# owensgroup/rtx_nerf

Hardware: AMD Instinct MI355X
Metric: Mrays/sec rendered (NeRF inference render, traverse->sample->MLP->composite) (higher is better)
Workload: dtype f16; 1 GPU; 800x800 inference render, 128^3 grid (procedural Lego stand-in occupancy, 5.3% cells), 8x128 ReLU MLP + Composite-Frequency encoding, 32 samples/segment, 4 hemisphere poses, seeded random fp16 weights; parallelism=single GPU, trace_mode=dda+mip, segments_per_frame_local_max=3152993

## Files before the change

### rtx_nerf_amd/csrc/mlp.hip

```cpp
#include "common.h"

#include <cmath>
#include <cstdlib>
#include <cstring>
#include <mutex>
#include <type_traits>
#include <vector>

#include "mlp_internal.h"

namespace {

#ifndef RTXN_SHARE_DIR
#define RTXN_SHARE_DIR 1
#endif
using rtxn::stage;

struct FwdArgs {
  const uint8_t* packed;
  int n_hidden;
  int out_act;
  const float* input;
  long n;
  const float* start;
  const float* end;
  const float* seg_view;
  const int* total_segments;
  long max_segments;
  _Float16* out_half;
  float4* radiance;
  float* t_vals;
};

struct Enc16Dims { int PD, PF, DD, DF, E, k0; };
__host__ __device__ inline int enc16_feature(const Enc16Dims& d, int u, int g) {
  const int FBD = (d.DF + 3) / 4, FBP = (d.PF + 3) / 4, ND = d.DD * FBD, NP = d.PD * FBP;
  const int width = 2 * (d.PD * d.PF + d.DD * d.DF);
  const int D = u >> 1, ph = u & 1;
  if (D < ND) { const int dd = D / FBD, f = FBD * g + D % FBD; return f < d.DF ? 2 * d.PD * d.PF + (dd * d.DF + f) * 2 + ph : -1; }
  if (D < ND + NP) { const int v = D - ND, dim = v / FBP, f = FBP * g + v % FBP; return f < d.PF ? (dim * d.PF + f) * 2 + ph : -1; }
  const int feat = width + 4 * (2 * (D - ND - NP) + ph) + g;
  return feat < d.E ? feat : -1;
}

__global__ void pack16_kernel(const _Float16* __restrict__ params, _Float16* __restrict__ packed, int W, int n_hidden, Enc16Dims d) {
  const int RT = W / 16, KS = W / 32, KS0 = d.k0 / 32, E = d.E;
  const long l0 = (long)KS0 * RT * 512, hid = (long)KS * RT * 512, outl = 4L * KS * 512;
  const long total = l0 + (long)(n_hidden - 1) * hid + outl;
  for (long e = (long)blockIdx.x * blockDim.x + threadIdx.x; e < total; e += (long)gridDim.x * blockDim.x) {
    int layer;
    long q = e;
    if (q < l0) layer = 0;
    else {
      q -= l0;
      layer = 1 + (int)(q / hid);
      if (layer >= n_hidden) { layer = n_hidden; q -= (long)(n_hidden - 1) * hid; } else q -= (long)(layer - 1) * hid;
    }
// ... 56 lines not shown
      const int feat = rtxn::perm_feature(kk, h, j);
      if (row < rows && feat < in_w) v = params[src_base(layer) + (long)row * in_w + feat];
    } else {
      const int ks_count = layer == n_hidden ? 1 : W / 16;
      const int kk = (int)(chunk % ks_count), rt = (int)(chunk / ks_count);
      const int col = 32 * rt + r;
      const int row = rtxn::perm_feature(kk, h, j);
      if (row < rows && col < in_w) v = params[src_base(layer) + (long)row * in_w + col];
    }
    packed[e] = v;
  }
}

template <int PD, int PF, int DD, int DF>
struct EncSpec16 {
  static constexpr int FBP = (PF + 3) / 4, FBD = (DF + 3) / 4;
  static_assert(FBP >= 1 && FBP <= 3 && FBD >= 1 && FBD <= 3, "octave_unit is written for 1-3 octaves per block");
  static constexpr int enc_width = 2 * (PD * PF + DD * DF);
  static constexpr int enc_padded = (enc_width + 15) / 16 * 16;
  static constexpr int ND = DD * FBD, NP = PD * FBP;
  static constexpr int NPADW = (enc_padded - enc_width + 7) / 8;
  static constexpr int n_dwords = ND + NP + NPADW;
  static constexpr int k0 = (n_dwords + 3) / 4 * 32;
  static_assert(ND <= 8, "direction dwords are placed before the pipeline starts: k-steps 0 and 1 only");
};

template <int NK>
__device__ __forceinline__ void octave_unit(float xg, int (&d)[3]) {
  float t, u, sn, cs;
  if constexpr (NK == 3) {
    asm volatile(
        "v_fract_f32 %3, %7\n\t"
        "v_sin_f32 %5, %3\n\t"
        "v_cos_f32 %6, %3\n\t"
        "s_nop 0\n\t"
        "v_cvt_pk_f16_f32 %0, %5, %6\n\t"
        "v_add_f32 %3, %5, %5\n\t"
        "v_mul_f32 %4, %3, %6\n\t"
        "v_fma_f32 %6, -%3, %5, 1.0\n\t"
// ... 40 lines not shown
template <int PD, int PF, int DD, int DF>
__device__ __forceinline__ void share_direction16(const float (&dir_g)[DD], int lane, int (&dirs)[DirShare16<PD, PF, DD, DF>::n_dwords]) {
  constexpr int FBD = EncSpec16<PD, PF, DD, DF>::FBD;
  const int c = lane & 15;
  float xs = dir_g[0];
#pragma unroll
  for (int dd = 1; dd < DD; ++dd) xs = c == dd ? dir_g[dd] : xs;
  int d[3];
  octave_unit<FBD>(xs, d);
#pragma unroll
  for (int dd = 0; dd < DD; ++dd)
#pragma unroll
    for (int k = 0; k < FBD; ++k) dirs[dd * FBD + k] = __builtin_amdgcn_ds_bpermute(4 * ((lane & 48) + dd), d[k]);
}

template <class ES, int PD, int PF, int DD, int DF, int KS0, int NB, int CT, bool SHARE>
__device__ __forceinline__ void encode_layer0_input(const float (&xq)[CT][5], const int (&dirs)[CT / 2][DirShare16<PD, PF, DD, DF>::n_dwords],
                                                    half8 (&bf)[NB][CT]) {
#pragma unroll
  for (int ct = 0; ct < CT; ++ct) {
    rtxn::int4v t[KS0];
#pragma unroll
    for (int kk = 0; kk < KS0; ++kk)
#pragma unroll
      for (int e = 0; e < 4; ++e) {
        const int D = 4 * kk + e;
        t[kk][e] = (D >= ES::ND + ES::NP && D < ES::n_dwords) ? 0x3c003c00 : 0;
      }
    if constexpr (SHARE) {
#pragma unroll
      for (int D = 0; D < ES::ND; ++D) t[D / 4][D % 4] = dirs[ct / 2][D];
    } else {
#pragma unroll
      for (int dd = 0; dd < DD; ++dd) {
        int d[3];
        octave_unit<ES::FBD>(xq[ct][PD + dd], d);
#pragma unroll
        for (int k = 0; k < ES::FBD; ++k) t[(dd * ES::FBD + k) / 4][(dd * ES::FBD + k) % 4] = d[k];
      }
    }
#pragma unroll
    for (int dim = 0; dim < PD; ++dim) {
      int d[3];
      octave_unit<ES::FBP>(xq[ct][dim], d);
#pragma unroll
      for (int k = 0; k < ES::FBP; ++k) t[(ES::ND + ES::FBP * dim + k) / 4][(ES::ND + ES::FBP * dim + k) % 4] = d[k];
    }
#pragma unroll
    for (int kk = 0; kk < KS0; ++kk) bf[kk][ct] = __builtin_bit_cast(half8, t[kk]);
    if constexpr (SHARE) asm volatile("" : "+v"(bf[0][ct]));
  }
}

#ifdef RTXN_STAMPS
constexpr int kStampTiles = 4, kStampSlots = 24;
__device__ unsigned g_stamps[8 * kStampTiles * kStampSlots];
#define RTXN_STAMP(k)                                                                                     \
  do {                                                                                                    \
    if (blockIdx.x == 0 && tile_it >= 2 && tile_it < 2 + kStampTiles) {                                   \
      const unsigned t_ = (unsigned)__builtin_amdgcn_s_memtime();                                         \
      if (lane == 0) stamp_lds[(wave_u * kStampTiles + (tile_it - 2)) * kStampSlots + (k)] = t_;          \
    }                                                                                                     \
  } while (0)
#else
#define RTXN_STAMP(k)
#endif
// ... 27 lines not shown
  } else {
    n_tiles = (int)((a.n + TILE - 1) / TILE);
  }
  n_tiles = __builtin_amdgcn_readfirstlane(n_tiles);
  const int tile_step = (int)gridDim.x;
  if ((int)blockIdx.x >= n_tiles) return;

  const int n_layers = a.n_hidden + 1;
  auto layer_off = [&](int l) -> unsigned { return l == 0 ? 0u : (unsigned)L0_BYTES + (unsigned)(l - 1) * HID_BYTES; };
  const int grp = wave_u >> 2;
  const int n_hid = n_layers - 2;
  stage<L0_BYTES, THREADS>(a.packed, smem, tid);
  stage<OUT_BYTES, THREADS>(a.packed + layer_off(n_layers - 1), smem + L0_BYTES, tid);
  int qs = 0;

  const float pos_scale = 0.5f * (float)(1u << (ES::FBP * g)), dir_scale = 0.5f * (float)(1u << (ES::FBD * g));
  float xq[CT][5];
  auto sample_of = [&](int tile, int ct, bool& valid) -> long {
    if (IN_MODE == 1) {
      const long seg = (long)tile * TILE_SEGS + wave_u * 2 + (ct >> 1);
      valid = seg < total_seg;
      return seg * 32 + 16 * (ct & 1) + c;
    }
    const long sidx = (long)tile * TILE + wave_u * 64 + ct * 16 + c;
    valid = sidx < a.n;
    return sidx;
  };
  typedef float f3v __attribute__((ext_vector_type(3)));
  typedef float f2v __attribute__((ext_vector_type(2)));
  f3v raw_s[CT / 2], raw_e[CT / 2];
  f2v raw_v[CT / 2];
// ... 17 lines not shown
        const long sidx = valid_in ? samp_in : 0;
#pragma unroll
        for (int k = 0; k < 5; ++k) raw_x[ct][k] = a.input[5 * sidx + k];
      }
    }
  };
  auto form_inputs = [&]() {
#pragma unroll
    for (int ct = 0; ct < CT; ++ct) {
      if (IN_MODE == 1) {
        const int sgi = ct >> 1;
        const float t = (float)(16 * (ct & 1) + c) * (1.0f / 32);
#pragma unroll
        for (int k = 0; k < 3; ++k) {
          const float og = raw_s[sgi][k];
          xq[ct][k] = fmaf(t, raw_e[sgi][k] - og, og) * pos_scale;
        }
        xq[ct][3] = raw_v[sgi][0] * dir_scale;
        xq[ct][4] = raw_v[sgi][1] * dir_scale;
      } else {
#pragma unroll
        for (int k = 0; k < 5; ++k) xq[ct][k] = raw_x[ct][k] * (k < PD ? pos_scale : dir_scale);
      }
    }
  };
  fetch_inputs((int)blockIdx.x);

  if (grp == 1) {
    if (n_hid > 0) {
      rtxn::StageJob sj0{a.packed + layer_off(1), smem + RES_BYTES, HID_BYTES / 1024};
      rtxn::stage_chunk<0, 8>(sj0, wave_u, lane);
      rtxn::stage_chunk<1, 8>(sj0, wave_u, lane);
      rtxn::stage_chunk<2, 8>(sj0, wave_u, lane);
      rtxn::stage_chunk<3, 8>(sj0, wave_u, lane);
    }
    rtxn::staged_barrier();
  }
  for (int tile = (int)blockIdx.x; tile < n_tiles; tile += tile_step) {
    const bool more = tile + tile_step < n_tiles;
    RTXN_STAMP(0);
    form_inputs();
    if (IN_MODE == 1 && OUT_MODE == 1 && a.t_vals) {
      int lane_t = lane;
      asm volatile("" : "+v"(lane_t));
      const long seg = (long)tile * TILE_SEGS + wave_u * 2 + (lane_t >> 5);
      if (seg < total_seg) a.t_vals[seg * 32 + (lane_t & 31)] = (float)((lane_t & 31) + 1) * (1.0f / 32);
    }
    constexpr bool SHARE = RTXN_SHARE_DIR && IN_MODE == 1 && DirShare16<PD, PF, DD, DF>::possible;
    int dirs[CT / 2][DirShare16<PD, PF, DD, DF>::n_dwords];
    if constexpr (SHARE) {
#pragma unroll
      for (int sg = 0; sg < CT / 2; ++sg) {
        float dg[DD];
#pragma unroll
        for (int dd = 0; dd < DD; ++dd) dg[dd] = xq[2 * sg][PD + dd];
        share_direction16<PD, PF, DD, DF>(dg, lane, dirs[sg]);
      }
    }
    half8 bf[NB][CT], bg[NB][CT];
    rtxn::floatx4 acc2[2][CT];
    rtxn::StageJob sj;
    auto begin_stage = [&](int l) -> const uint8_t* {
      rtxn::staged_barrier();
      const bool hidden = l > 0 && l < n_layers - 1;
      const uint8_t* cur = l == 0 ? smem : (hidden ? smem + RES_BYTES + (qs % 3) * HID_BYTES : smem + L0_BYTES);
      const int h0 = l == 0 ? 0 : (hidden ? l - 1 : n_hid);
      int lk = l + 1 + grp, inst = qs - h0;
      bool exists = true;
      if (lk >= n_layers) { lk -= n_layers; inst += n_hid; exists = more; }
      const bool fetch = exists && lk > 0 && lk < n_layers - 1;
      sj.g = a.packed + (unsigned)__builtin_amdgcn_readfirstlane((int)layer_off(fetch ? lk : 0));
      sj.lds = smem + RES_BYTES + (unsigned)__builtin_amdgcn_readfirstlane(((inst + lk - 1) % 3) * HID_BYTES);
      sj.nfrags = __builtin_amdgcn_readfirstlane(fetch ? HID_BYTES / 1024 : 0);
// ... 51 lines not shown
          samp = seg * 32 + (lane_e & 31);
        } else {
          samp = (long)tile * TILE + wave_u * 64 + lane_e;
          valid = samp < a.n;
        }
        if (valid) {
          half4v o;
#pragma unroll
          for (int e = 0; e < 4; ++e) o[e] = (_Float16)(a.out_act == RTXN_ACT_SIGMOID ? rtxn::sigmoidf_fast(z[e]) : z[e]);
          if (OUT_MODE == 3) *reinterpret_cast<half4v*>(a.out_half + samp * 4) = o;
          else a.radiance[samp] = make_float4((float)o[0], (float)o[1], (float)o[2], (float)o[3]);
        }
      }
    };
    {
      encode_layer0_input<ES, PD, PF, DD, DF, KS0, NB, CT, SHARE>(xq, dirs, bf);
      RTXN_STAMP(1);
      const uint8_t* w = begin_stage(0);
      RTXN_STAMP(2);
      rtxn::pipe_layer16<RT, KS0, NB, CT, false>(w, sj, bf, bg, acc2, wave_u, lane);
      RTXN_STAMP(3);
    }
    int l = 1;
    for (; l + 1 < n_layers - 1; l += 2) {
      const uint8_t* w = begin_stage(l);
      RTXN_STAMP(2 + 2 * l);
      rtxn::pipe_layer16<RT, KS, NB, CT, true>(w, sj, bg, bf, acc2, wave_u, lane);
      RTXN_STAMP(3 + 2 * l);
      w = begin_stage(l + 1);
      RTXN_STAMP(4 + 2 * l);
      rtxn::pipe_layer16<RT, KS, NB, CT, true>(w, sj, bf, bg, acc2, wave_u, lane);
      RTXN_STAMP(5 + 2 * l);
    }
    if (l < n_layers - 1) {
      const uint8_t* w = begin_stage(l);
// ... 45 lines not shown
  if (IN_MODE == 1) {
    total_seg = *a.total_segments;
    if (total_seg > a.max_segments) total_seg = a.max_segments;
    n_tiles = (int)((total_seg + 7) / 8);
  } else {
    n_tiles = (int)((a.n + 255) / 256);
  }
  n_tiles = __builtin_amdgcn_readfirstlane(n_tiles);
  if ((int)blockIdx.x >= n_tiles) return;
  const int tile_step = (int)gridDim.x;
  const int my_tiles = (n_tiles - (int)blockIdx.x + tile_step - 1) / tile_step;
  const int n_chunks = 4 + 4 * (a.n_hidden - 1) + 1;
  const int g_end = my_tiles * n_chunks;
  int gq = 0;

  const float pos_scale = 0.5f * (float)(1u << (ES::FBP * g)), dir_scale = 0.5f * (float)(1u << (ES::FBD * g));
  float xq[CT][5];
  auto sample_of = [&](int tile, int ct, bool& valid) -> long {
    if (IN_MODE == 1) {
      const long seg = (long)tile * 8 + wave_u;
      valid = seg < total_seg;
      return seg * 32 + 16 * ct + c;
    }
    const long sidx = (long)tile * 256 + wave_u * 32 + 16 * ct + c;
    valid = sidx < a.n;
    return sidx;
  };
  typedef float f3v __attribute__((ext_vector_type(3)));
  typedef float f2v __attribute__((ext_vector_type(2)));
  f3v raw_s, raw_e;
  f2v raw_v;
// ... 13 lines not shown
        const long samp_in = sample_of(tile, ct, valid_in);
        const long sidx = valid_in ? samp_in : 0;
#pragma unroll
        for (int k = 0; k < 5; ++k) raw_x[ct][k] = a.input[5 * sidx + k];
      }
    }
  };
  auto form_inputs = [&]() {
#pragma unroll
    for (int ct = 0; ct < CT; ++ct) {
      if (IN_MODE == 1) {
        const float t = (float)(16 * ct + c) * (1.0f / 32);
#pragma unroll
        for (int k = 0; k < 3; ++k) {
          const float og = raw_s[k];
          xq[ct][k] = fmaf(t, raw_e[k] - og, og) * pos_scale;
        }
        xq[ct][3] = raw_v[0] * dir_scale;
        xq[ct][4] = raw_v[1] * dir_scale;
      } else {
#pragma unroll
        for (int k = 0; k < 5; ++k) xq[ct][k] = raw_x[ct][k] * (k < PD ? pos_scale : dir_scale);
      }
    }
  };
  auto chunk_src = [&](int gi, int& size) -> unsigned {
    const int i = gi % n_chunks;
    if (i < 4) { size = L0_CHUNK; return (unsigned)i * L0_CHUNK; }
    if (i < n_chunks - 1) { size = HID_CHUNK; return 4u * L0_CHUNK + (unsigned)(i - 4) * HID_CHUNK; }
    size = OUT_CHUNK;
    return 4u * L0_CHUNK + (unsigned)(n_chunks - 5) * HID_CHUNK;
  };
  auto issue = [&](int gi) {
    int size;
    const unsigned off = chunk_src(gi, size);
    stage512(a.packed + off, smem + (gi % 3) * kSlot256, size, tid);
  };
// ... 22 lines not shown
      int lane_t = lane;
      asm volatile("" : "+v"(lane_t));
      const long seg = (long)tile * 8 + wave_u;
      if (seg < total_seg && lane_t < 32) a.t_vals[seg * 32 + lane_t] = (float)(lane_t + 1) * (1.0f / 32);
    }
    constexpr bool SHARE = RTXN_SHARE_DIR && IN_MODE == 1 && DirShare16<PD, PF, DD, DF>::possible;
    int dirs[1][DirShare16<PD, PF, DD, DF>::n_dwords];
    if constexpr (SHARE) {
      float dg[DD];
#pragma unroll
      for (int dd = 0; dd < DD; ++dd) dg[dd] = xq[0][PD + dd];
      share_direction16<PD, PF, DD, DF>(dg, lane, dirs[0]);
    }
    half8 bf[NB][CT], bg[NB][CT];
    rtxn::floatx4 acc2[2][CT];
    encode_layer0_input<ES, PD, PF, DD, DF, KS0, NB, CT, SHARE>(xq, dirs, bf);
    chunk_in_tile = 0;
    prefetch_tile = tile + tile_step < n_tiles ? tile + tile_step : -1;

    auto layer = [&](auto ks_tag, auto pend_tag, half8 (&in)[NB][CT], half8 (&out)[NB][CT]) {
      constexpr int KSL = decltype(ks_tag)::value;
      constexpr bool PEND0 = decltype(pend_tag)::value;
      const uint8_t* w = next_chunk();
      rtxn::pipe_chunk16<KSL, NB, CT, 4, 0, PEND0>(w, sj, in, out, acc2, wave_u, lane);
      w = next_chunk();
      rtxn::pipe_chunk16<KSL, NB, CT, 4, 4, true>(w, sj, in, out, acc2, wave_u, lane);
      w = next_chunk();
      rtxn::pipe_chunk16<KSL, NB, CT, 4, 8, true>(w, sj, in, out, acc2, wave_u, lane);
      w = next_chunk();
      rtxn::pipe_chunk16<KSL, NB, CT, 4, 12, true>(w, sj, in, out, acc2, wave_u, lane);
    };
// ... 425 lines not shown
```

### rtx_nerf_amd/csrc/mlp_internal.h

```cpp
#pragma once
#include "common.h"

typedef _Float16 half8 __attribute__((ext_vector_type(8)));
typedef _Float16 half4v __attribute__((ext_vector_type(4)));
typedef _Float16 half2v __attribute__((ext_vector_type(2)));
typedef float floatx16 __attribute__((ext_vector_type(16)));
typedef float float2v __attribute__((ext_vector_type(2)));
typedef short short2v __attribute__((ext_vector_type(2)));

struct rtxn_mlp {
  rtxn_mlp_config cfg;
  int enc_width;
  int enc_padded;
  int k0;
  long n_params;
  int variant;
  int reserved_cus;
  void* packed;
  size_t packed_bytes;
  void* packed_train;
  size_t packed_train_bytes;
  void* packed_t;
  size_t packed_t_bytes;
  int inference_ready;
// ... 223 lines not shown
    convert_unit16<NB, CT, RTI, P0>(acc, dst);
    convert_units16<NB, CT, RTI, P0 + 1, P1>(acc, dst);
  }
}
template <int NB, int CT, int RTI, int U, int KK>
__device__ __forceinline__ void convert_slice16(const floatx4 (&acc)[CT], half8 (&dst)[NB][CT]) {
  constexpr int p0 = KK * U < 2 * CT ? KK * U : 2 * CT, p1 = (KK + 1) * U < 2 * CT ? (KK + 1) * U : 2 * CT;
  convert_units16<NB, CT, RTI, p0, p1>(acc, dst);
}

#define RTXN_M16(ACC, B, C) "v_mfma_f32_16x16x32_f16 %[" ACC "], %[a], %[" B "], " C "\n\t"
#define RTXN_CVT16(U) "v_cvt_pk_f16_f32 %[r" U "], %[x" U "], %[y" U "]\n\t"
#define RTXN_MAX16(U) "v_pk_max_i16 %[r" U "], %[r" U "], 0\n\t"
#define RTXN_UNIT16(U) RTXN_CVT16(U) RTXN_MAX16(U)
#define RTXN_IN16 [a] "v"(a), [b0] "v"(b0), [b1] "v"(b1)
#define RTXN_PAIR16_CASES(M0, M1, ACC0, ACC1)                                                                                          \
  if constexpr (NUP == 0) asm volatile(M0 M1 : ACC0, ACC1 : RTXN_IN16);                                                                  \
  else if constexpr (NUP == 1) asm volatile(M0 RTXN_CVT16("0") M1 RTXN_MAX16("0") : ACC0, ACC1, RTXN_UOUT(0, 0) : RTXN_IN16, RTXN_UIN(0, 0)); \
  else if constexpr (NUP == 2)                                                                                                    \
    asm volatile(M0 RTXN_UNIT16("0") M1 RTXN_UNIT16("1") : ACC0, ACC1, RTXN_UOUT(0, 0), RTXN_UOUT(1, 1) : RTXN_IN16, RTXN_UIN(0, 0), RTXN_UIN(1, 1)); \
  else                                                                                                                            \
    asm volatile(M0 RTXN_UNIT16("0") RTXN_UNIT16("1") M1 RTXN_UNIT16("2") RTXN_UNIT16("3")                                         \
                 : ACC0, ACC1, RTXN_UOUT(0, 0), RTXN_UOUT(1, 1), RTXN_UOUT(2, 2), RTXN_UOUT(3, 3)                                         \
                 : RTXN_IN16, RTXN_UIN(0, 0), RTXN_UIN(1, 1), RTXN_UIN(2, 2), RTXN_UIN(3, 3));
template <bool ZERO, int NUP>
__device__ __forceinline__ void pair16(floatx4& acc0, floatx4& acc1, const half8& a, const half8& b0, const half8& b1,
                                       int (&r)[NUP > 0 ? NUP : 1], const float (&x)[NUP > 0 ? NUP : 1], const float (&y)[NUP > 0 ? NUP : 1]) {
  static_assert(NUP == 0 || NUP == 1 || NUP == 2 || NUP == 4, "unit pattern not written");
  if constexpr (ZERO) {
    RTXN_PAIR16_CASES(RTXN_M16("c0", "b0", "0"), RTXN_M16("c1", "b1", "0"), [c0] "=&v"(acc0), [c1] "=&v"(acc1))
  } else {
    RTXN_PAIR16_CASES(RTXN_M16("c0", "b0", "%[c0]"), RTXN_M16("c1", "b1", "%[c1]"), [c0] "+v"(acc0), [c1] "+v"(acc1))
  }
}
template <int NB, int CT, int RTI, int P0, int NU, bool ZERO, int PAIR>
struct PairRun16 {
  static constexpr int NPAIR = CT / 2;
  static constexpr int u0 = (NU * PAIR + NPAIR - 1) / NPAIR, u1 = (NU * (PAIR + 1) + NPAIR - 1) / NPAIR, NUP = u1 - u0;
  __device__ static __forceinline__ void run(const half8& a, const half8 (&b)[CT], floatx4 (&acc)[CT], const floatx4 (&fin)[CT],
                                             half8 (&dst)[NB][CT]) {
    int r[NUP > 0 ? NUP : 1];
    float x[NUP > 0 ? NUP : 1], y[NUP > 0 ? NUP : 1];
#pragma unroll
    for (int i = 0; i < NUP; ++i) {
      const int P = P0 + u0 + i;
      x[i] = fin[P / 2][2 * (P % 2)];
      y[i] = fin[P / 2][2 * (P % 2) + 1];
    }
    pair16<ZERO, NUP>(acc[2 * PAIR], acc[2 * PAIR + 1], a, b[2 * PAIR], b[2 * PAIR + 1], r, x, y);
#pragma unroll
    for (int i = 0; i < NUP; ++i) {
      const int P = P0 + u0 + i, ct = P / 2, e = P % 2;
      int4v t = __builtin_bit_cast(int4v, dst[RTI >> 1][ct]);
      t[2 * (RTI & 1) + e] = r[i];
      dst[RTI >> 1][ct] = __builtin_bit_cast(half8, t);
    }
    if constexpr (PAIR + 1 < NPAIR) PairRun16<NB, CT, RTI, P0, NU, ZERO, PAIR + 1>::run(a, b, acc, fin, dst);
  }
};
template <int NB, int CT, int RTI, int P0, int P1, bool ZERO>
__device__ __forceinline__ void mfma_convert_step16(const half8& a, const half8 (&b)[CT], floatx4 (&acc)[CT], const floatx4 (&fin)[CT],
                                                    half8 (&dst)[NB][CT]) {
  static_assert(CT % 2 == 0, "MFMAs go in pairs");
  PairRun16<NB, CT, RTI, P0, (P1 > P0 ? P1 - P0 : 0), ZERO, 0>::run(a, b, acc, fin, dst);
}
template <int CT, int U, int KK>
struct UnitRange16 {
  static constexpr int p0 = KK * U < 2 * CT ? KK * U : 2 * CT, p1 = (KK + 1) * U < 2 * CT ? (KK + 1) * U : 2 * CT;
};

template <int RT, int KS, int NB, int CT, bool PEND, int I>
struct PipeStep16 {
  static constexpr int D = RTXN_PIPE16, N = (RT ? RT : 1) * KS;
  static constexpr int U = (2 * CT + KS - 1) / KS;
  static constexpr int WIN = KS - 1 > 1 ? KS - 1 : 1;
  static constexpr int UP = (2 * CT + WIN - 1) / WIN;
  static constexpr int WAVES = RTXN_NW;
  static constexpr int CHUNKS = N < 32 / WAVES ? N : 32 / WAVES;
  __device__ static __forceinline__ void run(unsigned addr, half8 (&bf)[NB][CT], half8 (&nbf)[NB][CT], half8 (&ring)[D],
                                             floatx4 (&acc)[2][CT], const StageJob& sj, int wave_u, int lane) {
    constexpr int rt = I / KS, kk = I % KS, cur = rt & 1;
    constexpr int outstanding = (N - 1 - I) < (D - 1) ? (N - 1 - I) : (D - 1);
#if RTXN_PRIO_BANDS
#if RTXN_PRIO_BANDS == 1
    if constexpr (kk == 0 && RT >= 4 && rt % (RT / 4) == 0) asm volatile("s_setprio %0" ::"n"(3 - rt / (RT / 4)));
#elif RTXN_PRIO_BANDS == 2
    if constexpr (kk == 0 && RT >= 2 && rt % (RT / 2) == 0) asm volatile("s_setprio %0" ::"n"(1 - rt / (RT / 2)));
#elif RTXN_PRIO_BANDS == 3
    if constexpr (kk == 0 && RT >= 4 && rt % (RT / 4) == 0) asm volatile("s_setprio %0" ::"n"(rt / (RT / 4)));
#endif
#endif
    lds_wait_insn<outstanding>();
    if constexpr (rt > 0) {
      using R = UnitRange16<CT, U, kk>;
      mfma_convert_step16<NB, CT, rt - 1, R::p0, R::p1, kk == 0>(ring[I % D], bf[kk], acc[cur], acc[cur ^ 1], nbf);
    } else if constexpr (PEND && kk < WIN) {
      using R = UnitRange16<CT, UP, kk>;
      mfma_convert_step16<NB, CT, 2 * KS - 1, R::p0, R::p1, kk == 0>(ring[I % D], bf[kk], acc[cur], acc[1], bf);
    } else {
      mfma_convert_step16<NB, CT, 0, 0, 0, kk == 0>(ring[I % D], bf[kk], acc[cur], acc[cur], nbf);
    }
    __builtin_amdgcn_sched_barrier(0);
    if constexpr (I + D < N) lds_read_frag<(I + D) * 1024>(ring[I % D], addr);
    if constexpr (I < CHUNKS) {
      stage_chunk<I, WAVES>(sj, wave_u, lane);
      __builtin_amdgcn_sched_barrier(0);
    }
    if constexpr (I + 1 < N) PipeStep16<RT, KS, NB, CT, PEND, I + 1>::run(addr, bf, nbf, ring, acc, sj, wave_u, lane);
  }
};

template <int RT, int KS, int NB, int CT, bool PEND>
__device__ __forceinline__ void pipe_layer16(const uint8_t* lds_buf, const StageJob& sj, half8 (&bf)[NB][CT], half8 (&nbf)[NB][CT],
                                             floatx4 (&acc)[2][CT], int wave_u, int lane) {
  constexpr int D = RTXN_PIPE16, N = (RT ? RT : 1) * KS;
  static_assert(D >= 1 && D <= 4, "ring depth");
  static_assert(RT % 2 == 0, "the pending row tile must land in acc[1] and be the odd tile of its pair");
  static_assert(CT >= 2, "a unit must never read the accumulator of the MFMA issued just before it");
  static_assert(!PEND || KS >= 2, "the pending tile's fragment is first read at k-step KS-1; it is written during k-steps < KS-1");
  static_assert(NB >= KS, "fragment set too small");
  static_assert(N * 1024 <= 65535 + 1024, "fragment offsets must fit the 16-bit ds offset");
  half8 ring[D];
  const unsigned addr = (unsigned)(uintptr_t)(const __attribute__((address_space(3))) uint8_t*)lds_buf + lane * 16;
  lds_read_frag<0>(ring[0], addr);
  if constexpr (D > 1 && N > 1) lds_read_frag<1024>(ring[1 % D], addr);
  if constexpr (D > 2 && N > 2) lds_read_frag<2048>(ring[2 % D], addr);
  if constexpr (D > 3 && N > 3) lds_read_frag<3072>(ring[3 % D], addr);
  PipeStep16<RT, KS, NB, CT, PEND, 0>::run(addr, bf, nbf, ring, acc, sj, wave_u, lane);
  if constexpr (RT == 0) mfma_results_settle(acc[0]);
}

template <int KS, int NB, int CT, int NR, int RT0, bool PEND, int I>
struct PipeStep16c {
  static constexpr int D = RTXN_PIPE16, N = NR * KS, WAVES = 8;
  static constexpr int SPAN = KS - 1;
  static constexpr int U = (2 * CT + SPAN - 1) / SPAN;
  static constexpr int WIN = KS - 1 > 1 ? KS - 1 : 1;
  static constexpr int UP = (2 * CT + WIN - 1) / WIN;
  static constexpr int CHUNKS = 4;
  __device__ static __forceinline__ void run(unsigned addr, half8 (&in)[NB][CT], half8 (&out)[NB][CT], half8 (&ring)[D],
                                             floatx4 (&acc)[2][CT], const StageJob& sj, int wave_u, int lane) {
    constexpr int r = I / KS, kk = I % KS, cur = r & 1;
    constexpr int outstanding = (N - 1 - I) < (D - 1) ? (N - 1 - I) : (D - 1);
#if RTXN_PRIO_BANDS256
// ... 80 lines not shown
```

Measured before the change: 38.19 Mrays/s.

## Compute direction contribution of layer 0 once per segment as MFMA bias

Restructures the first MLP layer. All samples in a segment share one view direction, so the direction-encoding part of the layer-0 matmul is now computed once per segment pair by a separate small MFMA pass and fed in as the C-operand bias. The main pipeline then only runs over the position k-steps. The position encoding is also repacked into two fixed k-steps laid out for 3x10 octaves, with per-dimension scales and a lane-dependent slot. This is meant to cut redundant layer-0 MFMA work and encoding ALU, at the cost of hard-coded dimension assumptions, DPP shuffles, and hazard nops.

New measurement: 39.51 Mrays/s (median of 6 runs). +3.5%, better.

```diff
diff --git a/rtx_nerf_amd/csrc/mlp.hip b/rtx_nerf_amd/csrc/mlp.hip
--- a/rtx_nerf_amd/csrc/mlp.hip
+++ b/rtx_nerf_amd/csrc/mlp.hip
@@ -33,14 +33,21 @@
 };
 
 struct Enc16Dims { int PD, PF, DD, DF, E, k0; };
+__host__ __device__ inline int pos16_start(int dim, int g) {
+  return dim == 1 ? (g == 0 ? 0 : g == 1 ? 2 : g == 2 ? 4 : 7) : (g == 0 ? 0 : g == 1 ? 3 : g == 2 ? 6 : 8);
+}
+__host__ __device__ inline int pos16_count(int dim, int g) { return dim == 1 ? (g < 2 ? 2 : 3) : (g < 2 ? 3 : 2); }
 __host__ __device__ inline int enc16_feature(const Enc16Dims& d, int u, int g) {
-  const int FBD = (d.DF + 3) / 4, FBP = (d.PF + 3) / 4, ND = d.DD * FBD, NP = d.PD * FBP;
+  const int FBD = (d.DF + 3) / 4, ND = d.DD * FBD;
   const int width = 2 * (d.PD * d.PF + d.DD * d.DF);
+  const int NPADW = (d.E - width + 7) / 8, KSD = (ND + NPADW + 3) / 4;
   const int D = u >> 1, ph = u & 1;
   if (D < ND) { const int dd = D / FBD, f = FBD * g + D % FBD; return f < d.DF ? 2 * d.PD * d.PF + (dd * d.DF + f) * 2 + ph : -1; }
-  if (D < ND + NP) { const int v = D - ND, dim = v / FBP, f = FBP * g + v % FBP; return f < d.PF ? (dim * d.PF + f) * 2 + ph : -1; }
-  const int feat = width + 4 * (2 * (D - ND - NP) + ph) + g;
-  return feat < d.E ? feat : -1;
+  if (D < ND + NPADW) { const int feat = width + 4 * (2 * (D - ND) + ph) + g; return feat < d.E ? feat : -1; }
+  const int s = D - 4 * KSD;
+  if (s < 0 || s >= 8) return -1;
+  const int dim = s < 6 ? s >> 1 : (s == 7 ? 2 : (g < 2 ? 0 : 1)), k = s < 6 ? (s & 1) : 2;
+  return k < pos16_count(dim, g) ? (dim * d.PF + pos16_start(dim, g) + k) * 2 + ph : -1;
 }
 
 __global__ void pack16_kernel(const _Float16* __restrict__ params, _Float16* __restrict__ packed, int W, int n_hidden, Enc16Dims d) {
@@ -127,15 +134,18 @@
 
 template <int PD, int PF, int DD, int DF>
 struct EncSpec16 {
-  static constexpr int FBP = (PF + 3) / 4, FBD = (DF + 3) / 4;
-  static_assert(FBP >= 1 && FBP <= 3 && FBD >= 1 && FBD <= 3, "octave_unit is written for 1-3 octaves per block");
+  static_assert(PD == 3 && PF == 10, "the position block is laid out for 3 dimensions x 10 octaves (pos16_start)");
+  static constexpr int FBD = (DF + 3) / 4;
+  static_assert(FBD >= 1 && FBD <= 3, "octave_unit is written for 1-3 octaves per block");
   static constexpr int enc_width = 2 * (PD * PF + DD * DF);
   static constexpr int enc_padded = (enc_width + 15) / 16 * 16;
-  static constexpr int ND = DD * FBD, NP = PD * FBP;
+  static constexpr int ND = DD * FBD;
   static constexpr int NPADW = (enc_padded - enc_width + 7) / 8;
-  static constexpr int n_dwords = ND + NP + NPADW;
-  static constexpr int k0 = (n_dwords + 3) / 4 * 32;
-  static_assert(ND <= 8, "direction dwords are placed before the pipeline starts: k-steps 0 and 1 only");
+  static constexpr int KSD = (ND + NPADW + 3) / 4, KSP = 2;
+  static constexpr int POS0 = 4 * KSD;
+  static constexpr int n_dwords = POS0 + 8;
+  static constexpr int k0 = (KSD + KSP) * 32;
+  static_assert(KSD <= 2, "direction dwords are placed before the pipeline starts: k-steps 0 and 1 only");
 };
 
 template <int NK>
@@ -206,9 +216,10 @@
     for (int k = 0; k < FBD; ++k) dirs[dd * FBD + k] = __builtin_amdgcn_ds_bpermute(4 * ((lane & 48) + dd), d[k]);
 }
 
-template <class ES, int PD, int PF, int DD, int DF, int KS0, int NB, int CT, bool SHARE>
+template <class ES, int PD, int PF, int DD, int DF, int KS0, int NB, int CT, bool SHARE, bool POS_ONLY = false>
 __device__ __forceinline__ void encode_layer0_input(const float (&xq)[CT][5], const int (&dirs)[CT / 2][DirShare16<PD, PF, DD, DF>::n_dwords],
-                                                    half8 (&bf)[NB][CT]) {
+                                                    bool lo, half8 (&bf)[NB][CT]) {
+  static_assert(KS0 == ES::KSD + ES::KSP, "k-steps as staged");
 #pragma unroll
   for (int ct = 0; ct < CT; ++ct) {
     rtxn::int4v t[KS0];
@@ -217,9 +228,10 @@
 #pragma unroll
       for (int e = 0; e < 4; ++e) {
         const int D = 4 * kk + e;
-        t[kk][e] = (D >= ES::ND + ES::NP && D < ES::n_dwords) ? 0x3c003c00 : 0;
+        t[kk][e] = (D >= ES::ND && D < ES::ND + ES::NPADW) ? 0x3c003c00 : 0;
       }
-    if constexpr (SHARE) {
+    if constexpr (POS_ONLY) {
+    } else if constexpr (SHARE) {
 #pragma unroll
       for (int D = 0; D < ES::ND; ++D) t[D / 4][D % 4] = dirs[ct / 2][D];
     } else {
@@ -231,17 +243,47 @@
         for (int k = 0; k < ES::FBD; ++k) t[(dd * ES::FBD + k) / 4][(dd * ES::FBD + k) % 4] = d[k];
       }
     }
-#pragma unroll
-    for (int dim = 0; dim < PD; ++dim) {
-      int d[3];
-      octave_unit<ES::FBP>(xq[ct][dim], d);
-#pragma unroll
-      for (int k = 0; k < ES::FBP; ++k) t[(ES::ND + ES::FBP * dim + k) / 4][(ES::ND + ES::FBP * dim + k) % 4] = d[k];
-    }
-#pragma unroll
-    for (int kk = 0; kk < KS0; ++kk) bf[kk][ct] = __builtin_bit_cast(half8, t[kk]);
-    if constexpr (SHARE) asm volatile("" : "+v"(bf[0][ct]));
-  }
+    int p[PD][3];
+#pragma unroll
+    for (int dim = 0; dim < PD; ++dim) octave_unit<3>(xq[ct][dim], p[dim]);
+    int slot[8];
+#pragma unroll
+    for (int dim = 0; dim < PD; ++dim) slot[2 * dim] = p[dim][0], slot[2 * dim + 1] = p[dim][1];
+    slot[6] = lo ? p[0][2] : p[1][2];
+    slot[7] = p[2][2];
+#pragma unroll
+    for (int i = 0; i < 8; ++i) t[(ES::POS0 + i) / 4][(ES::POS0 + i) % 4] = slot[i];
+    if constexpr (POS_ONLY) {
+#pragma unroll
+      for (int kk = 0; kk < ES::KSP; ++kk) bf[kk][ct] = __builtin_bit_cast(half8, t[ES::KSD + kk]);
+    } else {
+#pragma unroll
+      for (int kk = 0; kk < KS0; ++kk) bf[kk][ct] = __builtin_bit_cast(half8, t[kk]);
+    }
+    if constexpr (SHARE && !POS_ONLY) asm volatile("" : "+v"(bf[0][ct]));
+  }
+}
+
+template <class ES, int PD, int DD, int CT>
+__device__ __forceinline__ void encode_direction_pair(const float (&xq)[CT][5], int c, half8 (&bd)[ES::KSD]) {
+  rtxn::int4v t[ES::KSD];
+#pragma unroll
+  for (int kk = 0; kk < ES::KSD; ++kk)
+#pragma unroll
+    for (int e = 0; e < 4; ++e) {
+      const int D = 4 * kk + e;
+      t[kk][e] = (D >= ES::ND && D < ES::ND + ES::NPADW) ? 0x3c003c00 : 0;
+    }
+#pragma unroll
+  for (int dd = 0; dd < DD; ++dd) {
+    const float x = (c & 1) ? xq[2][PD + dd] : xq[0][PD + dd];
+    int d[3];
+    octave_unit<ES::FBD>(x, d);
+#pragma unroll
+    for (int k = 0; k < ES::FBD; ++k) t[(dd * ES::FBD + k) / 4][(dd * ES::FBD + k) % 4] = d[k];
+  }
+#pragma unroll
+  for (int kk = 0; kk < ES::KSD; ++kk) bd[kk] = __builtin_bit_cast(half8, t[kk]);
 }
 
 #ifdef RTXN_STAMPS
@@ -299,7 +341,9 @@
   stage<OUT_BYTES, THREADS>(a.packed + layer_off(n_layers - 1), smem + L0_BYTES, tid);
   int qs = 0;
 
-  const float pos_scale = 0.5f * (float)(1u << (ES::FBP * g)), dir_scale = 0.5f * (float)(1u << (ES::FBD * g));
+  const float dir_scale = 0.5f * (float)(1u << (ES::FBD * g));
+  const float pos_scale[3] = {0.5f * (float)(1u << pos16_start(0, g)), 0.5f * (float)(1u << pos16_start(1, g)),
+                              0.5f * (float)(1u << pos16_start(2, g))};
   float xq[CT][5];
   auto sample_of = [&](int tile, int ct, bool& valid) -> long {
     if (IN_MODE == 1) {
@@ -347,13 +391,13 @@
 #pragma unroll
         for (int k = 0; k < 3; ++k) {
           const float og = raw_s[sgi][k];
-          xq[ct][k] = fmaf(t, raw_e[sgi][k] - og, og) * pos_scale;
+          xq[ct][k] = fmaf(t, raw_e[sgi][k] - og, og) * pos_scale[k];
         }
         xq[ct][3] = raw_v[sgi][0] * dir_scale;
         xq[ct][4] = raw_v[sgi][1] * dir_scale;
       } else {
 #pragma unroll
-        for (int k = 0; k < 5; ++k) xq[ct][k] = raw_x[ct][k] * (k < PD ? pos_scale : dir_scale);
+        for (int k = 0; k < 5; ++k) xq[ct][k] = raw_x[ct][k] * (k < PD ? pos_scale[k < PD ? k : 0] : dir_scale);
       }
     }
   };
@@ -379,17 +423,10 @@
       const long seg = (long)tile * TILE_SEGS + wave_u * 2 + (lane_t >> 5);
       if (seg < total_seg) a.t_vals[seg * 32 + (lane_t & 31)] = (float)((lane_t & 31) + 1) * (1.0f / 32);
     }
-    constexpr bool SHARE = RTXN_SHARE_DIR && IN_MODE == 1 && DirShare16<PD, PF, DD, DF>::possible;
+    constexpr bool BIAS = RTXN_SHARE_DIR && IN_MODE == 1;
     int dirs[CT / 2][DirShare16<PD, PF, DD, DF>::n_dwords];
-    if constexpr (SHARE) {
-#pragma unroll
-      for (int sg = 0; sg < CT / 2; ++sg) {
-        float dg[DD];
-#pragma unroll
-        for (int dd = 0; dd < DD; ++dd) dg[dd] = xq[2 * sg][PD + dd];
-        share_direction16<PD, PF, DD, DF>(dg, lane, dirs[sg]);
-      }
-    }
+    half8 bd[ES::KSD];
+    if constexpr (BIAS) encode_direction_pair<ES, PD, DD, CT>(xq, c, bd);
     half8 bf[NB][CT], bg[NB][CT];
     rtxn::floatx4 acc2[2][CT];
     rtxn::StageJob sj;
@@ -471,11 +508,17 @@
       }
     };
     {
-      encode_layer0_input<ES, PD, PF, DD, DF, KS0, NB, CT, SHARE>(xq, dirs, bf);
+      encode_layer0_input<ES, PD, PF, DD, DF, KS0, NB, CT, false, BIAS>(xq, dirs, g < 2, bf);
       RTXN_STAMP(1);
       const uint8_t* w = begin_stage(0);
       RTXN_STAMP(2);
-      rtxn::pipe_layer16<RT, KS0, NB, CT, false>(w, sj, bf, bg, acc2, wave_u, lane);
+      if constexpr (BIAS) {
+        rtxn::floatx4 bias[RT];
+        rtxn::dir_bias16<RT, ES::KSD, KS0>(w, bd, bias, lane);
+        rtxn::pipe_layer16<RT, ES::KSP, NB, CT, false, KS0, ES::KSD, true>(w, sj, bf, bg, acc2, wave_u, lane, bias);
+      } else {
+        rtxn::pipe_layer16<RT, KS0, NB, CT, false>(w, sj, bf, bg, acc2, wave_u, lane);
+      }
       RTXN_STAMP(3);
     }
     int l = 1;
@@ -551,7 +594,9 @@
   const int g_end = my_tiles * n_chunks;
   int gq = 0;
 
-  const float pos_scale = 0.5f * (float)(1u << (ES::FBP * g)), dir_scale = 0.5f * (float)(1u << (ES::FBD * g));
+  const float dir_scale = 0.5f * (float)(1u << (ES::FBD * g));
+  const float pos_scale[3] = {0.5f * (float)(1u << pos16_start(0, g)), 0.5f * (float)(1u << pos16_start(1, g)),
+                              0.5f * (float)(1u << pos16_start(2, g))};
   float xq[CT][5];
   auto sample_of = [&](int tile, int ct, bool& valid) -> long {
     if (IN_MODE == 1) {
@@ -595,13 +640,13 @@
 #pragma unroll
         for (int k = 0; k < 3; ++k) {
           const float og = raw_s[k];
-          xq[ct][k] = fmaf(t, raw_e[k] - og, og) * pos_scale;
+          xq[ct][k] = fmaf(t, raw_e[k] - og, og) * pos_scale[k];
         }
         xq[ct][3] = raw_v[0] * dir_scale;
         xq[ct][4] = raw_v[1] * dir_scale;
       } else {
 #pragma unroll
-        for (int k = 0; k < 5; ++k) xq[ct][k] = raw_x[ct][k] * (k < PD ? pos_scale : dir_scale);
+        for (int k = 0; k < 5; ++k) xq[ct][k] = raw_x[ct][k] * (k < PD ? pos_scale[k < PD ? k : 0] : dir_scale);
       }
     }
   };
@@ -654,7 +699,7 @@
     }
     half8 bf[NB][CT], bg[NB][CT];
     rtxn::floatx4 acc2[2][CT];
-    encode_layer0_input<ES, PD, PF, DD, DF, KS0, NB, CT, SHARE>(xq, dirs, bf);
+    encode_layer0_input<ES, PD, PF, DD, DF, KS0, NB, CT, SHARE>(xq, dirs, g < 2, bf);
     chunk_in_tile = 0;
     prefetch_tile = tile + tile_step < n_tiles ? tile + tile_step : -1;
 
diff --git a/rtx_nerf_amd/csrc/mlp_internal.h b/rtx_nerf_amd/csrc/mlp_internal.h
--- a/rtx_nerf_amd/csrc/mlp_internal.h
+++ b/rtx_nerf_amd/csrc/mlp_internal.h
@@ -261,31 +261,36 @@
 #define RTXN_MAX16(U) "v_pk_max_i16 %[r" U "], %[r" U "], 0\n\t"
 #define RTXN_UNIT16(U) RTXN_CVT16(U) RTXN_MAX16(U)
 #define RTXN_IN16 [a] "v"(a), [b0] "v"(b0), [b1] "v"(b1)
-#define RTXN_PAIR16_CASES(M0, M1, ACC0, ACC1)                                                                                          \
-  if constexpr (NUP == 0) asm volatile(M0 M1 : ACC0, ACC1 : RTXN_IN16);                                                                  \
-  else if constexpr (NUP == 1) asm volatile(M0 RTXN_CVT16("0") M1 RTXN_MAX16("0") : ACC0, ACC1, RTXN_UOUT(0, 0) : RTXN_IN16, RTXN_UIN(0, 0)); \
+#define RTXN_IN16Z [a] "v"(a), [b0] "v"(b0), [b1] "v"(b1), [z] "v"(z)
+#define RTXN_PAIR16_CASES(M0, M1, ACC0, ACC1, IN)                                                                                      \
+  if constexpr (NUP == 0) asm volatile(M0 M1 : ACC0, ACC1 : IN);                                                                         \
+  else if constexpr (NUP == 1) asm volatile(M0 RTXN_CVT16("0") M1 RTXN_MAX16("0") : ACC0, ACC1, RTXN_UOUT(0, 0) : IN, RTXN_UIN(0, 0));        \
   else if constexpr (NUP == 2)                                                                                                    \
-    asm volatile(M0 RTXN_UNIT16("0") M1 RTXN_UNIT16("1") : ACC0, ACC1, RTXN_UOUT(0, 0), RTXN_UOUT(1, 1) : RTXN_IN16, RTXN_UIN(0, 0), RTXN_UIN(1, 1)); \
+    asm volatile(M0 RTXN_UNIT16("0") M1 RTXN_UNIT16("1") : ACC0, ACC1, RTXN_UOUT(0, 0), RTXN_UOUT(1, 1) : IN, RTXN_UIN(0, 0), RTXN_UIN(1, 1)); \
   else                                                                                                                            \
     asm volatile(M0 RTXN_UNIT16("0") RTXN_UNIT16("1") M1 RTXN_UNIT16("2") RTXN_UNIT16("3")                                         \
                  : ACC0, ACC1, RTXN_UOUT(0, 0), RTXN_UOUT(1, 1), RTXN_UOUT(2, 2), RTXN_UOUT(3, 3)                                         \
-                 : RTXN_IN16, RTXN_UIN(0, 0), RTXN_UIN(1, 1), RTXN_UIN(2, 2), RTXN_UIN(3, 3));
-template <bool ZERO, int NUP>
+                 : IN, RTXN_UIN(0, 0), RTXN_UIN(1, 1), RTXN_UIN(2, 2), RTXN_UIN(3, 3));
+template <bool ZERO, int NUP, bool BZ = false>
 __device__ __forceinline__ void pair16(floatx4& acc0, floatx4& acc1, const half8& a, const half8& b0, const half8& b1,
-                                       int (&r)[NUP > 0 ? NUP : 1], const float (&x)[NUP > 0 ? NUP : 1], const float (&y)[NUP > 0 ? NUP : 1]) {
+                                       int (&r)[NUP > 0 ? NUP : 1], const float (&x)[NUP > 0 ? NUP : 1], const float (&y)[NUP > 0 ? NUP : 1],
+                                       const floatx4& z = floatx4{}) {
   static_assert(NUP == 0 || NUP == 1 || NUP == 2 || NUP == 4, "unit pattern not written");
-  if constexpr (ZERO) {
-    RTXN_PAIR16_CASES(RTXN_M16("c0", "b0", "0"), RTXN_M16("c1", "b1", "0"), [c0] "=&v"(acc0), [c1] "=&v"(acc1))
+  static_assert(!(ZERO && BZ), "one C source");
+  if constexpr (BZ) {
+    RTXN_PAIR16_CASES("s_nop 1\n\t" RTXN_M16("c0", "b0", "%[z]"), RTXN_M16("c1", "b1", "%[z]"), [c0] "=&v"(acc0), [c1] "=&v"(acc1), RTXN_IN16Z)
+  } else if constexpr (ZERO) {
+    RTXN_PAIR16_CASES(RTXN_M16("c0", "b0", "0"), RTXN_M16("c1", "b1", "0"), [c0] "=&v"(acc0), [c1] "=&v"(acc1), RTXN_IN16)
   } else {
-    RTXN_PAIR16_CASES(RTXN_M16("c0", "b0", "%[c0]"), RTXN_M16("c1", "b1", "%[c1]"), [c0] "+v"(acc0), [c1] "+v"(acc1))
-  }
-}
-template <int NB, int CT, int RTI, int P0, int NU, bool ZERO, int PAIR>
+    RTXN_PAIR16_CASES(RTXN_M16("c0", "b0", "%[c0]"), RTXN_M16("c1", "b1", "%[c1]"), [c0] "+v"(acc0), [c1] "+v"(acc1), RTXN_IN16)
+  }
+}
+template <int NB, int CT, int RTI, int P0, int NU, bool ZERO, int PAIR, bool BZ = false>
 struct PairRun16 {
   static constexpr int NPAIR = CT / 2;
   static constexpr int u0 = (NU * PAIR + NPAIR - 1) / NPAIR, u1 = (NU * (PAIR + 1) + NPAIR - 1) / NPAIR, NUP = u1 - u0;
   __device__ static __forceinline__ void run(const half8& a, const half8 (&b)[CT], floatx4 (&acc)[CT], const floatx4 (&fin)[CT],
-                                             half8 (&dst)[NB][CT]) {
+                                             half8 (&dst)[NB][CT], const floatx4 (&bz)[NPAIR]) {
     int r[NUP > 0 ? NUP : 1];
     float x[NUP > 0 ? NUP : 1], y[NUP > 0 ? NUP : 1];
 #pragma unroll
@@ -294,7 +299,7 @@
       x[i] = fin[P / 2][2 * (P % 2)];
       y[i] = fin[P / 2][2 * (P % 2) + 1];
     }
-    pair16<ZERO, NUP>(acc[2 * PAIR], acc[2 * PAIR + 1], a, b[2 * PAIR], b[2 * PAIR + 1], r, x, y);
+    pair16<ZERO, NUP, BZ>(acc[2 * PAIR], acc[2 * PAIR + 1], a, b[2 * PAIR], b[2 * PAIR + 1], r, x, y, bz[PAIR]);
 #pragma unroll
     for (int i = 0; i < NUP; ++i) {
       const int P = P0 + u0 + i, ct = P / 2, e = P % 2;
@@ -302,21 +307,21 @@
       t[2 * (RTI & 1) + e] = r[i];
       dst[RTI >> 1][ct] = __builtin_bit_cast(half8, t);
     }
-    if constexpr (PAIR + 1 < NPAIR) PairRun16<NB, CT, RTI, P0, NU, ZERO, PAIR + 1>::run(a, b, acc, fin, dst);
-  }
-};
-template <int NB, int CT, int RTI, int P0, int P1, bool ZERO>
+    if constexpr (PAIR + 1 < NPAIR) PairRun16<NB, CT, RTI, P0, NU, ZERO, PAIR + 1, BZ>::run(a, b, acc, fin, dst, bz);
+  }
+};
+template <int NB, int CT, int RTI, int P0, int P1, bool ZERO, bool BZ = false>
 __device__ __forceinline__ void mfma_convert_step16(const half8& a, const half8 (&b)[CT], floatx4 (&acc)[CT], const floatx4 (&fin)[CT],
-                                                    half8 (&dst)[NB][CT]) {
+                                                    half8 (&dst)[NB][CT], const floatx4 (&bz)[CT / 2] = {}) {
   static_assert(CT % 2 == 0, "MFMAs go in pairs");
-  PairRun16<NB, CT, RTI, P0, (P1 > P0 ? P1 - P0 : 0), ZERO, 0>::run(a, b, acc, fin, dst);
+  PairRun16<NB, CT, RTI, P0, (P1 > P0 ? P1 - P0 : 0), ZERO, 0, BZ>::run(a, b, acc, fin, dst, bz);
 }
 template <int CT, int U, int KK>
 struct UnitRange16 {
   static constexpr int p0 = KK * U < 2 * CT ? KK * U : 2 * CT, p1 = (KK + 1) * U < 2 * CT ? (KK + 1) * U : 2 * CT;
 };
 
-template <int RT, int KS, int NB, int CT, bool PEND, int I>
+template <int RT, int KS, int NB, int CT, bool PEND, int I, int KSTR = KS, int KOFF = 0, bool BIAS = false>
 struct PipeStep16 {
   static constexpr int D = RTXN_PIPE16, N = (RT ? RT : 1) * KS;
   static constexpr int U = (2 * CT + KS - 1) / KS;
@@ -324,10 +329,14 @@
   static constexpr int UP = (2 * CT + WIN - 1) / WIN;
   static constexpr int WAVES = RTXN_NW;
   static constexpr int CHUNKS = N < 32 / WAVES ? N : 32 / WAVES;
+  static constexpr int NBIAS = BIAS ? RT : 1;
+  __host__ __device__ static constexpr int frag_off(int i) { return ((i / KS) * KSTR + KOFF + i % KS) * 1024; }
   __device__ static __forceinline__ void run(unsigned addr, half8 (&bf)[NB][CT], half8 (&nbf)[NB][CT], half8 (&ring)[D],
-                                             floatx4 (&acc)[2][CT], const StageJob& sj, int wave_u, int lane) {
+                                             floatx4 (&acc)[2][CT], const StageJob& sj, int wave_u, int lane,
+                                             const floatx4 (&bias)[NBIAS], floatx4 (&bz)[CT / 2]) {
     constexpr int rt = I / KS, kk = I % KS, cur = rt & 1;
     constexpr int outstanding = (N - 1 - I) < (D - 1) ? (N - 1 - I) : (D - 1);
+    constexpr bool ZERO = kk == 0 && !BIAS, BZ = kk == 0 && BIAS;
 #if RTXN_PRIO_BANDS
 #if RTXN_PRIO_BANDS == 1
     if constexpr (kk == 0 && RT >= 4 && rt % (RT / 4) == 0) asm volatile("s_setprio %0" ::"n"(3 - rt / (RT / 4)));
@@ -337,44 +346,110 @@
     if constexpr (kk == 0 && RT >= 4 && rt % (RT / 4) == 0) asm volatile("s_setprio %0" ::"n"(rt / (RT / 4)));
 #endif
 #endif
+    if constexpr (BZ) {
+      static_assert(CT == 4, "two segments per wave");
+#pragma unroll
+      for (int e = 0; e < 4; ++e) {
+        float s0, s1;
+        asm volatile("v_mov_b32_dpp %0, %2 quad_perm:[0,0,2,2] row_mask:0xf bank_mask:0xf\n\t"
+                     "v_mov_b32_dpp %1, %2 quad_perm:[1,1,3,3] row_mask:0xf bank_mask:0xf"
+                     : "=&v"(s0), "=&v"(s1) : "v"(bias[rt][e]));
+        bz[0][e] = s0;
+        bz[1][e] = s1;
+      }
+    }
     lds_wait_insn<outstanding>();
     if constexpr (rt > 0) {
       using R = UnitRange16<CT, U, kk>;
-      mfma_convert_step16<NB, CT, rt - 1, R::p0, R::p1, kk == 0>(ring[I % D], bf[kk], acc[cur], acc[cur ^ 1], nbf);
+      mfma_convert_step16<NB, CT, rt - 1, R::p0, R::p1, ZERO, BZ>(ring[I % D], bf[kk], acc[cur], acc[cur ^ 1], nbf, bz);
     } else if constexpr (PEND && kk < WIN) {
       using R = UnitRange16<CT, UP, kk>;
-      mfma_convert_step16<NB, CT, 2 * KS - 1, R::p0, R::p1, kk == 0>(ring[I % D], bf[kk], acc[cur], acc[1], bf);
+      mfma_convert_step16<NB, CT, 2 * KS - 1, R::p0, R::p1, ZERO, BZ>(ring[I % D], bf[kk], acc[cur], acc[1], bf, bz);
     } else {
-      mfma_convert_step16<NB, CT, 0, 0, 0, kk == 0>(ring[I % D], bf[kk], acc[cur], acc[cur], nbf);
-    }
+      mfma_convert_step16<NB, CT, 0, 0, 0, ZERO, BZ>(ring[I % D], bf[kk], acc[cur], acc[cur], nbf, bz);
+    }
+    if constexpr (BIAS && kk == 1) asm volatile("" ::"v"(bz[0]), "v"(bz[1]));
     __builtin_amdgcn_sched_barrier(0);
-    if constexpr (I + D < N) lds_read_frag<(I + D) * 1024>(ring[I % D], addr);
+    if constexpr (I + D < N) lds_read_frag<frag_off(I + D)>(ring[I % D], addr);
     if constexpr (I < CHUNKS) {
       stage_chunk<I, WAVES>(sj, wave_u, lane);
       __builtin_amdgcn_sched_barrier(0);
     }
-    if constexpr (I + 1 < N) PipeStep16<RT, KS, NB, CT, PEND, I + 1>::run(addr, bf, nbf, ring, acc, sj, wave_u, lane);
-  }
-};
-
-template <int RT, int KS, int NB, int CT, bool PEND>
+    if constexpr (I + 1 < N)
+      PipeStep16<RT, KS, NB, CT, PEND, I + 1, KSTR, KOFF, BIAS>::run(addr, bf, nbf, ring, acc, sj, wave_u, lane, bias, bz);
+  }
+};
+
+template <int RT, int KS, int NB, int CT, bool PEND, int KSTR = KS, int KOFF = 0, bool BIAS = false>
 __device__ __forceinline__ void pipe_layer16(const uint8_t* lds_buf, const StageJob& sj, half8 (&bf)[NB][CT], half8 (&nbf)[NB][CT],
-                                             floatx4 (&acc)[2][CT], int wave_u, int lane) {
+                                             floatx4 (&acc)[2][CT], int wave_u, int lane,
+                                             const floatx4 (&bias)[PipeStep16<RT, KS, NB, CT, PEND, 0, KSTR, KOFF, BIAS>::NBIAS] = {}) {
+  using P = PipeStep16<RT, KS, NB, CT, PEND, 0, KSTR, KOFF, BIAS>;
   constexpr int D = RTXN_PIPE16, N = (RT ? RT : 1) * KS;
   static_assert(D >= 1 && D <= 4, "ring depth");
   static_assert(RT % 2 == 0, "the pending row tile must land in acc[1] and be the odd tile of its pair");
   static_assert(CT >= 2, "a unit must never read the accumulator of the MFMA issued just before it");
   static_assert(!PEND || KS >= 2, "the pending tile's fragment is first read at k-step KS-1; it is written during k-steps < KS-1");
+  static_assert(!BIAS || (KS >= 2 && !PEND && RT >= 4), "bias copies live one k-step past their MFMAs; dir_bias16's hazard distance");
   static_assert(NB >= KS, "fragment set too small");
-  static_assert(N * 1024 <= 65535 + 1024, "fragment offsets must fit the 16-bit ds offset");
+  static_assert(P::frag_off(N - 1) <= 65535, "fragment offsets must fit the 16-bit ds offset");
   half8 ring[D];
+  floatx4 bz[CT / 2];
   const unsigned addr = (unsigned)(uintptr_t)(const __attribute__((address_space(3))) uint8_t*)lds_buf + lane * 16;
-  lds_read_frag<0>(ring[0], addr);
-  if constexpr (D > 1 && N > 1) lds_read_frag<1024>(ring[1 % D], addr);
-  if constexpr (D > 2 && N > 2) lds_read_frag<2048>(ring[2 % D], addr);
-  if constexpr (D > 3 && N > 3) lds_read_frag<3072>(ring[3 % D], addr);
-  PipeStep16<RT, KS, NB, CT, PEND, 0>::run(addr, bf, nbf, ring, acc, sj, wave_u, lane);
+  lds_read_frag<P::frag_off(0)>(ring[0], addr);
+  if constexpr (D > 1 && N > 1) lds_read_frag<P::frag_off(1)>(ring[1 % D], addr);
+  if constexpr (D > 2 && N > 2) lds_read_frag<P::frag_off(2)>(ring[2 % D], addr);
+  if constexpr (D > 3 && N > 3) lds_read_frag<P::frag_off(3)>(ring[3 % D], addr);
+  P::run(addr, bf, nbf, ring, acc, sj, wave_u, lane, bias, bz);
   if constexpr (RT == 0) mfma_results_settle(acc[0]);
+}
+
+template <int RT, int KSD, int KS0, int P>
+struct DirBias16 {
+  static constexpr int NF = 2 * KSD;
+  static constexpr int frag_off(int f) { return ((2 * P + (f & 1)) * KS0 + (f >> 1)) * 1024; }
+  __device__ static __forceinline__ void read(half8 (&ring)[NF], unsigned addr) {
+    lds_read_frag<frag_off(0)>(ring[0], addr);
+    lds_read_frag<frag_off(1)>(ring[1], addr);
+    if constexpr (KSD > 1) {
+      lds_read_frag<frag_off(2)>(ring[2], addr);
+      lds_read_frag<frag_off(3)>(ring[3], addr);
+    }
+  }
+  __device__ static __forceinline__ void run(unsigned addr, const half8 (&bd)[KSD], floatx4 (&bias)[RT], half8 (&ring)[2][NF]) {
+    static_assert(KSD == 1 || KSD == 2, "statements written for one or two direction k-steps");
+    if constexpr (2 * P + 2 < RT) {
+      DirBias16<RT, KSD, KS0, P + 1>::read(ring[(P + 1) & 1], addr);
+      lds_wait_insn<NF>();
+    } else {
+      lds_wait_insn<0>();
+    }
+    const half8(&a)[NF] = ring[P & 1];
+#define RTXN_MB16(ACC, A, B, C) "v_mfma_f32_16x16x32_f16 %[" ACC "], %[" A "], %[" B "], " C "\n\t"
+    if constexpr (KSD == 1) {
+      asm volatile(RTXN_MB16("c0", "a0", "d0", "0") RTXN_MB16("c1", "a1", "d0", "0")
+                   : [c0] "=&v"(bias[2 * P]), [c1] "=&v"(bias[2 * P + 1])
+                   : [d0] "v"(bd[0]), [a0] "v"(a[0]), [a1] "v"(a[1]));
+    } else {
+      asm volatile(RTXN_MB16("c0", "a0", "d0", "0") RTXN_MB16("c1", "a1", "d0", "0")
+                   RTXN_MB16("c0", "a2", "d1", "%[c0]") RTXN_MB16("c1", "a3", "d1", "%[c1]")
+                   : [c0] "=&v"(bias[2 * P]), [c1] "=&v"(bias[2 * P + 1])
+                   : [d0] "v"(bd[0]), [d1] "v"(bd[1]), [a0] "v"(a[0]), [a1] "v"(a[1]), [a2] "v"(a[2]), [a3] "v"(a[3]));
+    }
+#undef RTXN_MB16
+    __builtin_amdgcn_sched_barrier(0);
+    if constexpr (2 * P + 2 < RT) DirBias16<RT, KSD, KS0, P + 1>::run(addr, bd, bias, ring);
+  }
+};
+template <int RT, int KSD, int KS0>
+__device__ __forceinline__ void dir_bias16(const uint8_t* lds_buf, const half8 (&bd)[KSD], floatx4 (&bias)[RT], int lane) {
+  static_assert(RT % 2 == 0 && RT >= 4, "row tiles in pairs; see the hazard note");
+  static_assert(((RT - 1) * KS0 + KSD - 1) * 1024 <= 65535, "fragment offsets must fit the 16-bit ds offset");
+  half8 ring[2][2 * KSD];
+  const unsigned addr = (unsigned)(uintptr_t)(const __attribute__((address_space(3))) uint8_t*)lds_buf + lane * 16;
+  DirBias16<RT, KSD, KS0, 0>::read(ring[0], addr);
+  DirBias16<RT, KSD, KS0, 0>::run(addr, bd, bias, ring);
+  asm volatile("s_nop 15\n\ts_nop 7" : "+v"(bias[0]), "+v"(bias[1]));
 }
 
 template <int KS, int NB, int CT, int NR, int RT0, bool PEND, int I>
```
